# araffin/srl-zoo

Hardware: AMD Instinct MI355X
Metric: images/sec (224x224x3) AE+VAE train step (higher is better)
Workload: dtype f32; 1 GPU; synthetic 224x224x3 obs, --losses autoencoder, custom_cnn, state-dim 200, bs=256 per GPU (512 frames fwd+bwd per step per GPU), Adam lr 0.005, normalised fp32 observations resident in HBM; global_batch=256, parallelism=dp1, rccl_ranks=1, devices=1

## Files before the change

### include/srlz.h

```cpp
#ifndef SRLZ_H
#define SRLZ_H

#include <stddef.h>
#include <stdint.h>

#ifdef __cplusplus
extern "C" {
#endif

typedef void* srlz_stream_t;

enum srlz_status {
  SRLZ_OK = 0,
  SRLZ_ERR_BAD_DESC = -1,
  SRLZ_ERR_WORKSPACE = -2,
  SRLZ_ERR_HIP = -3,
  SRLZ_ERR_NULL = -4
};

#define SRLZ_ABI_VERSION 104
int srlz_version(void);
const char* srlz_last_error(void);
int srlz_device_cus(void);

typedef struct {
  int n;
  int hi, wi;
  int ho, wo;
  int ksize;
  int stride;
  int pad;
  int transposed;
  int groups;
} srlz_conv64_desc;

size_t srlz_conv64_packed_floats(void);
int srlz_conv64_pack_weights(const float* w_ref, float* wpack_fwd, float* wpack_bwd,
                             const srlz_conv64_desc* d, srlz_stream_t stream);
int srlz_conv64_fwd_tiles(const srlz_conv64_desc* d);
int srlz_conv64_fwd(const float* x, const float* wpack_fwd, const float* bias, float* y, float* stats_partial,
                    const float* x_bnp, const srlz_conv64_desc* d, srlz_stream_t stream);
typedef struct {
  const float* y;
  const float* bnp;
  const float* sums;
  long long count;
  int training;
  float* dy_out;
} srlz_bn_bwd_operand;
int srlz_conv64_bwd_data(const float* dy, const float* wpack_bwd, float* dx, const srlz_bn_bwd_operand* dy_bn,
                         const srlz_conv64_desc* d, srlz_stream_t stream);
struct srlz_pool_desc_s;
int srlz_conv64_bwd_data_tiles(const srlz_conv64_desc* d);
int srlz_conv64_bwd_data_pool_sums(const float* dy, const float* wpack_bwd, float* dx, const float* pooled, const float* pool_bnp,
                                   const float* pool_y, const uint8_t* pool_argmax, const struct srlz_pool_desc_s* pd,
                                   float* bn_bwd_partial, const srlz_conv64_desc* d, srlz_stream_t stream);
int srlz_conv64_bwd_fused_supported(const srlz_conv64_desc* d);
int srlz_conv64_gather_pipe_supported(const srlz_conv64_desc* d, int backward_data);
size_t srlz_conv64_bwd_fused_workspace(const srlz_conv64_desc* d);
int srlz_conv64_bwd_fused_bn_rows(const srlz_conv64_desc* d);
int srlz_conv64_bwd_fused(const float* x, const float* x_bnp, const float* dy, const srlz_bn_bwd_operand* dy_bn,
                          const float* wpack_bwd, float* dx, float* dw_ref, float* dbias ,
                          float* x_bn_bwd_partial , void* ws, size_t ws_bytes, const srlz_conv64_desc* d,
                          srlz_stream_t stream);
int srlz_conv64_wino_supported(const srlz_conv64_desc* d);
size_t srlz_conv64_wino_packed_floats(void);
int srlz_conv64_wino_pack_weights(const float* w_ref, float* upack_fwd, float* upack_bwd, srlz_stream_t stream);
int srlz_conv64_wino_tiles(const srlz_conv64_desc* d);
int srlz_conv64_wino_fwd(const float* x, const float* upack_fwd, const float* bias , float* y,
                         float* stats_partial , const float* x_bnp ,
                         const srlz_conv64_desc* d, srlz_stream_t stream);
int srlz_conv64_wino_bwd_data(const float* dy, const float* upack_bwd, float* dx, const srlz_conv64_desc* d, srlz_stream_t stream);
int srlz_conv64_wino_bwd_data_rows(const srlz_conv64_desc* d);
int srlz_conv64_wino_bwd_data_pool_sums(const float* dy, const float* upack_bwd, float* dx, const float* pooled, const float* pool_bnp,
                                        const float* pool_y, const uint8_t* pool_argmax, const struct srlz_pool_desc_s* pd,
                                        float* bn_bwd_partial, const srlz_conv64_desc* d, srlz_stream_t stream);
size_t srlz_conv64_wino_bwd_weight_workspace(const srlz_conv64_desc* d);
int srlz_conv64_wino_bwd_weight(const float* x, const float* dy, float* dw_ref, void* ws, size_t ws_bytes, const srlz_conv64_desc* d,
                                srlz_stream_t stream);
size_t srlz_conv64_bwd_weight_workspace(const srlz_conv64_desc* d);
int srlz_conv64_bwd_weight(const float* x, const float* dy, float* dw_ref, float* dbias, const float* x_bnp ,
                           const srlz_bn_bwd_operand* dy_bn ,
                           void* ws, size_t ws_bytes, const srlz_conv64_desc* d, srlz_stream_t stream);

typedef struct {
  int n, hi, wi, ho, wo;
  int cin, cout;
  int ksize, stride, pad;
  int groups;
} srlz_convn_desc;
size_t srlz_convn_packed_floats(const srlz_convn_desc* d);
int srlz_convn_pack_weights(const float* w_ref, float* wpack, const srlz_convn_desc* d, srlz_stream_t stream);
int srlz_convn_fwd_tiles(const srlz_convn_desc* d);
int srlz_convn_fwd(const float* x, const float* wpack, float* y, float* stats_partial, const float* x_bnp,
                   const srlz_convn_desc* d, srlz_stream_t stream);

typedef struct {
  int n;
  int c;
  int himg, wimg;
  int hf, wf;
  int kind;
  int groups;
} srlz_skinny_desc;

int srlz_skinny_tiles(const srlz_skinny_desc* d);
int srlz_conv1_fwd(const float* x_nchw, const float* w_ref, float* y_nhwc, float* stats_partial,
                   const srlz_skinny_desc* d, srlz_stream_t stream);
int srlz_conv1_fwd_u8(const uint8_t* x_u8, const float* norm_lut, const float* w_ref, float* y_nhwc, float* stats_partial,
                      const srlz_skinny_desc* d, srlz_stream_t stream);
size_t srlz_skinny_bwd_weight_workspace(const srlz_skinny_desc* d);
// ... 291 lines not shown
```

### srl-zoo_amd/csrc/conv64.hip

```cpp
#include "conv64_tile.h"
#include <stdlib.h>

static int floordiv(int a, int b) { return (a >= 0) ? a / b : -((-a + b - 1) / b); }

int conv64::build_program(Prog* P, int gather, int stride, int pad, int N, int Hs, int Ws, int Hd, int Wd, int G) {
  if (stride != 1 && stride != 2) return -1;
  if (G < 1 || N % G != 0) return -1;
  N /= G;
  P->N = N; P->Hs = Hs; P->Ws = Ws; P->Hd = Hd; P->Wd = Wd;
  P->G = G;
  P->src_gstride = (long long)N * Hs * Ws * 64;
  P->dst_gstride = (long long)N * Hd * Wd * 64;
  int kcls[3], kd[3];
  if (gather) {
    P->ss = stride; P->ds = 1;
    for (int k = 0; k < 3; ++k) {
      int t = k - pad;
      int c = ((t % stride) + stride) % stride;
      kcls[k] = c; kd[k] = (t - c) / stride;
    }
  } else {
    P->ss = 1; P->ds = stride;
    for (int k = 0; k < 3; ++k) {
      int py = (((k - pad) % stride) + stride) % stride;
// ... 355 lines not shown
                                                                    const float* __restrict__ wpack,
                                                                    const float* __restrict__ bias,
                                                                    float* __restrict__ dst,
                                                                    float* __restrict__ stats_partial,
                                                                    const ConvProg P, int ntiles, const OpFuse src_fuse_all) {
  conv64_fwd_body<NW, BWD, 0>(src, wpack, bias, dst, stats_partial, P, ntiles, src_fuse_all, SRLZ_NO_POOLSUM);
}

template <int PSUM>
__global__ __launch_bounds__(256, 2) void conv64_dgrad_poolsum_kernel(const float* __restrict__ src,
                                                                     const float* __restrict__ wpack,
                                                                     float* __restrict__ dst,
                                                                     float* __restrict__ bn_bwd_partial, const ConvProg P,
                                                                     int ntiles, const PoolSum ps) {
  conv64_fwd_body<4, false, PSUM>(src, wpack, nullptr, dst, bn_bwd_partial, P, ntiles, SRLZ_NO_FUSE, ps);
}

__global__ void conv64_pack_kernel(const float* __restrict__ w_ref, float* __restrict__ pf, float* __restrict__ pb,
                                   int transposed) {
  const int id = blockIdx.x * blockDim.x + threadIdx.x;
  if (id >= NTAPS * 4096) return;
  const int tap = id >> 12, n = (id >> 6) & 63, k = id & 63;
  const int o = (tap * 64 + n) * 64 + ((((k >> 2) ^ (n & 15)) << 2) | (k & 3));
  const int fwd_idx = transposed ? ((k * 64 + n) * 9 + tap) : ((n * 64 + k) * 9 + tap);
  const int bwd_idx = transposed ? ((n * 64 + k) * 9 + tap) : ((k * 64 + n) * 9 + tap);
  if (pf) pf[o] = w_ref[fwd_idx];
  if (pb) pb[o] = w_ref[bwd_idx];
}

static int check_desc(const srlz_conv64_desc* d) {
  SRLZ_REQUIRE(d != nullptr, SRLZ_ERR_NULL, "conv64: null descriptor");
  SRLZ_REQUIRE(d->ksize == 3 && (d->stride == 1 || d->stride == 2) && d->n > 0, SRLZ_ERR_BAD_DESC,
               "conv64: only 3x3 stride 1/2 supported (k=%d s=%d)", d->ksize, d->stride);
  SRLZ_REQUIRE(d->groups >= 0 && (d->groups <= 1 || d->n % d->groups == 0), SRLZ_ERR_BAD_DESC,
               "conv64: n = %d is not a multiple of groups = %d", d->n, d->groups);
  int eho, ewo;
  if (!d->transposed) {
    eho = (d->hi + 2 * d->pad - 3) / d->stride + 1;
    ewo = (d->wi + 2 * d->pad - 3) / d->stride + 1;
  } else {
    eho = (d->hi - 1) * d->stride - 2 * d->pad + 3;
    ewo = (d->wi - 1) * d->stride - 2 * d->pad + 3;
  }
  SRLZ_REQUIRE(eho == d->ho && ewo == d->wo, SRLZ_ERR_BAD_DESC, "conv64: output size %dx%d inconsistent (expected %dx%d)",
               d->ho, d->wo, eho, ewo);
  return 0;
}

static size_t fwd_lds_bytes(const ConvProg& P) {
  return (size_t)(TM + P.span) * 256 + 16384 + (size_t)64 * rowtab_passes(TM + P.span) + TM * 4 + 256 * 4;
}

static int launch_fwd(const float* src, const float* wpack, const float* bias, float* dst, float* stats,
                      const ConvProg& P, hipStream_t st, const OpFuse src_fuse = SRLZ_NO_FUSE, const PoolSum* psum = nullptr) {
  const int ntiles = P.G * P.tpg;
  const size_t lds = fwd_lds_bytes(P);
  SRLZ_REQUIRE(lds <= 160 * 1024, SRLZ_ERR_BAD_DESC, "conv64: tile needs %zu bytes of LDS", lds);
  SRLZ_REQUIRE(fits_32bit_src_floats(P) && fits_32bit_dst_rowinfo(P) && fits_31bit_grid(P, TM + P.span), SRLZ_ERR_BAD_DESC, "conv64: a group of %d images of %d x %d -> %d x %d is beyond the tile tables' 32-bit offsets", P.N, P.Hs,
               P.Ws, P.Hd, P.Wd);
  if (psum) {
    SRLZ_REQUIRE(!src_fuse.y && !src_fuse.bnp && stats && !bias, SRLZ_ERR_BAD_DESC, "conv64: the pooled-block epilogue takes a plain operand");
    bool one_class = true;
    for (int t = 1; t < NTAPS; ++t) one_class = one_class && P.tdst[t] == P.tdst[0];
    if (one_class) {
      SRLZ_MAX_LDS(conv64_dgrad_poolsum_kernel<1>, lds);
      SRLZ_LAUNCH(conv64_dgrad_poolsum_kernel<1>, dim3(ntiles), dim3(256), lds, st, src, wpack, dst, stats, P, ntiles, *psum);
    } else {
      SRLZ_MAX_LDS(conv64_dgrad_poolsum_kernel<2>, lds);
      SRLZ_LAUNCH(conv64_dgrad_poolsum_kernel<2>, dim3(ntiles), dim3(256), lds, st, src, wpack, dst, stats, P, ntiles, *psum);
    }
    return 0;
  }
#define SRLZ_FWD_LAUNCH(NWV, BWDV)                                                                                          \
  do {                                                                                                                     \
    SRLZ_MAX_LDS((conv64_fwd_kernel<NWV, BWDV>), lds);                                                                      \
    SRLZ_LAUNCH((conv64_fwd_kernel<NWV, BWDV>), dim3(ntiles), dim3(NWV * 64), lds, st, src, wpack, bias, dst, stats,        \
                P, ntiles, src_fuse);                                                                                      \
  } while (0)
  if (src_fuse.y) {
    SRLZ_REQUIRE(fits_32bit_src_floats(P), SRLZ_ERR_BAD_DESC,
                 "conv64: a group's operand has %lld floats (the fused staging keeps 32-bit row offsets)", (long long)P.N * P.Hs * P.Ws * 64);
    SRLZ_FWD_LAUNCH(4, true);
  } else {
    if (!src_fuse.bnp && !bias && conv64::gather_pipe_ok(P)) return conv64::launch_gather_pipe(src, wpack, dst, stats, P, st);
    SRLZ_FWD_LAUNCH(4, false);
  }
#undef SRLZ_FWD_LAUNCH
  return 0;
}

}

int conv64::with_program(const srlz_conv64_desc* d, int backward_data, Prog* P) {
  if (int rc = check_desc(d)) return rc;
  const int G = d->groups > 1 ? d->groups : 1;
  const int rc = backward_data ? build_program(P, d->transposed, d->stride, d->pad, d->n, d->ho, d->wo, d->hi, d->wi, G)
                               : build_program(P, !d->transposed, d->stride, d->pad, d->n, d->hi, d->wi, d->ho, d->wo, G);
  SRLZ_REQUIRE(rc == 0, SRLZ_ERR_BAD_DESC, "conv64: cannot build a grid program for this descriptor");
  return 0;
}

extern "C" size_t srlz_conv64_packed_floats(void) { return (size_t)NTAPS * 4096; }

extern "C" int srlz_conv64_pack_weights(const float* w_ref, float* wpack_fwd, float* wpack_bwd,
                                        const srlz_conv64_desc* d, srlz_stream_t stream) {
  if (int rc = check_desc(d)) return rc;
  SRLZ_REQUIRE(w_ref, SRLZ_ERR_NULL, "conv64_pack: null weights");
  SRLZ_LAUNCH(conv64_pack_kernel, dim3((NTAPS * 4096 + 255) / 256), dim3(256), 0, as_stream(stream), w_ref, wpack_fwd, wpack_bwd,
              d->transposed);
  return 0;
}

extern "C" int srlz_conv64_fwd_tiles(const srlz_conv64_desc* d) {
  ConvProg P;
  if (conv64::with_program(d, 0, &P)) return -1;
  return P.G * P.tpg;
}

extern "C" int srlz_conv64_fwd(const float* x, const float* wpack_fwd, const float* bias, float* y,
                               float* stats_partial, const float* x_bnp, const srlz_conv64_desc* d,
                               srlz_stream_t stream) {
  ConvProg P;
  if (int rc = conv64::with_program(d, 0, &P)) return rc;
  SRLZ_REQUIRE(x && wpack_fwd && y, SRLZ_ERR_NULL, "conv64_fwd: null pointer");
  return launch_fwd(x, wpack_fwd, bias, y, stats_partial, P, as_stream(stream), OpFuse{x_bnp, nullptr, nullptr, 0.f, 0, nullptr});
}

extern "C" int srlz_conv64_bwd_data(const float* dy, const float* wpack_bwd, float* dx, const srlz_bn_bwd_operand* dy_bn,
                                    const srlz_conv64_desc* d, srlz_stream_t stream) {
  ConvProg P;
  if (int rc = conv64::with_program(d, 1, &P)) return rc;
  SRLZ_REQUIRE(dy && wpack_bwd && dx, SRLZ_ERR_NULL, "conv64_bwd_data: null pointer");
  OpFuse gf;
  if (int rc = make_bwd_fuse(&gf, dy_bn, "conv64_bwd_data")) return rc;
  return launch_fwd(dy, wpack_bwd, nullptr, dx, nullptr, P, as_stream(stream), gf);
}

extern "C" int srlz_conv64_bwd_data_tiles(const srlz_conv64_desc* d) {
  ConvProg P;
  if (conv64::with_program(d, 1, &P)) return -1;
  return P.G * P.tpg;
}

extern "C" int srlz_conv64_bwd_data_pool_sums(const float* dy, const float* wpack_bwd, float* dx, const float* pooled,
                                              const float* pool_bnp, const float* pool_y, const uint8_t* pool_argmax,
                                              const srlz_pool_desc* pd, float* bn_bwd_partial, const srlz_conv64_desc* d,
                                              srlz_stream_t stream) {
  ConvProg P;
  if (int rc = conv64::with_program(d, 1, &P)) return rc;
  SRLZ_REQUIRE(dy && wpack_bwd && dx && pooled && pool_bnp && pool_y && pool_argmax && pd && bn_bwd_partial, SRLZ_ERR_NULL,
               "conv64_bwd_data_pool_sums: null pointer");
  SRLZ_REQUIRE(pd->n == d->n && pd->hp == d->hi && pd->wp == d->wi && !pd->out_nchw &&
               (pd->groups > 1 ? pd->groups : 1) == (d->groups > 1 ? d->groups : 1), SRLZ_ERR_BAD_DESC,
               "conv64_bwd_data_pool_sums: the pooled map [%d,%d,%d] is not this layer's input [%d,%d,%d]", pd->n, pd->hp, pd->wp, d->n,
               d->hi, d->wi);
  const int G = d->groups > 1 ? d->groups : 1;
  PoolSum ps = {pooled, pool_bnp, pool_y, pool_argmax, (long long)(pd->n / G) * pd->h * pd->w * 64, pd->h, pd->w, pd->pool_pad};
  return launch_fwd(dy, wpack_bwd, nullptr, dx, bn_bwd_partial, P, as_stream(stream), SRLZ_NO_FUSE, &ps);
}

extern "C" int srlz_conv64_debug_program(const srlz_conv64_desc* d, int backward_data, int* out, int cap) {
  ConvProg P;
  if (int rc = conv64::with_program(d, backward_data, &P)) return rc;
  if (cap < 12 + 4 * NTAPS) return SRLZ_ERR_WORKSPACE;
  int i = 0;
  out[i++] = P.N; out[i++] = P.PH; out[i++] = P.PW; out[i++] = P.ss; out[i++] = P.Hs; out[i++] = P.Ws;
  out[i++] = P.ds; out[i++] = P.Hd; out[i++] = P.Wd; out[i++] = P.min_off; out[i++] = P.span; out[i++] = P.s2;
  for (int t = 0; t < NTAPS; ++t) { out[i++] = P.tsrc[t]; out[i++] = P.tdst[t]; out[i++] = P.toff[t]; out[i++] = P.tw[t]; }
  return i;
}
```

### srl-zoo_amd/csrc/conv64_pipe.hip

```cpp
#include "conv64_tile.h"

namespace {

constexpr int GP_THREADS = 512;
constexpr int GP_RP = GP_THREADS / 16;
constexpr int GP_BATCH = 6;
constexpr int GP_CORE = TM / GP_RP;

struct GatherRows {
  f32x4 v[GP_BATCH], yv[GP_BATCH];
  unsigned offs[GP_CORE];
  unsigned ok;
};

constexpr int GT_P = 8;
constexpr int GT_WORDS = GP_RP * GT_P;
template <bool SHIFTED>
__device__ __forceinline__ void gtab_build(unsigned* __restrict__ tab, const ConvProg& P, int qstart, int nrows) {
  int R = threadIdx.x;
  asm volatile("" : "+v"(R));
  if (R < GT_WORDS) {
    unsigned e = 0;
    if (R < nrows) e = src_entry<SHIFTED>(P, qstart + R, 2);
    tab[(R & (GP_RP - 1)) * GT_P + (R >> 5)] = e;
// ... 612 lines not shown
    float* X = As0;
    if (wk == 1) {
#pragma unroll
      for (int r = 0; r < 16; ++r) X[((wave & 3) * 16 + r) * 64 + lane] = aw3[0][r];
    }
    __syncthreads();
    if (wk == 0) {
#pragma unroll
      for (int r = 0; r < 16; ++r) aw3[0][r] += X[((wave & 3) * 16 + r) * 64 + lane];
      put(aw3[0], 8, wmi, wnj);
    }
    __syncthreads();
    float* red = As0;
    *(f32x4*)(red + (tid >> 4) * 64 + (tid & 15) * 4) = bs4;
    __syncthreads();
    if (tid < 64) {
      float t = 0.f;
#pragma unroll
      for (int r = 0; r < GP_RP; ++r) t += red[r * 64 + tid];
      out[NTAPS * 4096 + tid] = t;
    }
  }
}

constexpr int BNZ_BLOCKS = 64;
__global__ __launch_bounds__(256) void conv64_bnpart_zero_scale_kernel(const float* __restrict__ x, const float* __restrict__ x_bnp,
                                                                      const float* __restrict__ da, float* __restrict__ bnpart,
                                                                      long long pixels, int bn_rows, int first_row) {
  const int g = blockIdx.y;
  x_bnp += g * 256;
  x += (size_t)g * pixels * 64;
  da += (size_t)g * pixels * 64;
  const int c4 = threadIdx.x & 15;
  const auto [mean, invstd, sc, sh] = load_bn_quads(x_bnp, c4);
  unsigned zmask = 0;
#pragma unroll
  for (int j = 0; j < 4; ++j) zmask |= (bnpart_zero_scale(sc[j], sh[j]) ? 1u : 0u) << j;
  double s1[4] = {0.0, 0.0, 0.0, 0.0}, s2[4] = {0.0, 0.0, 0.0, 0.0};
  if (__syncthreads_or(zmask != 0)) {
    for (long long pix = (long long)blockIdx.x * 16 + (threadIdx.x >> 4); pix < pixels; pix += (long long)gridDim.x * 16) {
      const f32x4 v = *(const f32x4*)(x + pix * 64 + c4 * 4);
      const f32x4 d = *(const f32x4*)(da + pix * 64 + c4 * 4);
#pragma unroll
      for (int j = 0; j < 4; ++j)
        if (((zmask >> j) & 1u) && v[j] * sc[j] + sh[j] > 0.f) {
          s1[j] += (double)d[j];
          s2[j] += (double)(d[j] * ((v[j] - mean[j]) * invstd[j]));
        }
    }
  }
  bn_bwd_combine_store(s1, s2, bnpart + ((size_t)g * bn_rows + first_row + blockIdx.x) * 128);
}

}

constexpr int GATHER_PIPE_MIN_TILES_PER_GROUP = 256;
bool conv64::gather_pipe_ok(const Prog& P) {
  if (P.tpg < GATHER_PIPE_MIN_TILES_PER_GROUP) return false;
  return taps_grouped_4221(P) && P.G <= 2 && fits_32bit_buffer_bytes(P) && TM + P.span <= GP_RP * GP_BATCH && GP_RP <= P.PHW &&
         -P.min_off <= P.PHW;
}

int conv64::launch_gather_pipe(const float* src, const float* wpack, float* dst, float* stats, const Prog& P, hipStream_t st) {
  const int ntiles = P.G * P.tpg;
  int pgrid = 2 * srlz_device_cus();
  if (pgrid > ntiles) pgrid = ntiles;
  pgrid &= ~7;
  if (pgrid < 8) pgrid = 8;
  const size_t plds = (size_t)(TM + P.span) * 256 + 16384 + 6 * TM * 4 + GT_WORDS * 4 + 8 * 64 * 4;
  SRLZ_MAX_LDS(conv64_gather_pipe_kernel, plds);
  SRLZ_LAUNCH(conv64_gather_pipe_kernel, dim3(pgrid), dim3(GP_THREADS), plds, st, src, wpack, dst, stats, ConvProg{P}, ntiles);
  return 0;
}

static bool fused_bwd_ok(const ConvProg& P) {
  const bool reach = P.toff[4] >= 0 && P.toff[5] >= 0 && P.toff[4] < FB_REACH1 && P.toff[5] < FB_REACH1 && P.toff[8] >= 0 &&
                     P.toff[8] <= FB_REACH3;
  return taps_grouped_4221(P) && P.G <= 2 && P.min_off == 0 && fits_32bit_buffer_bytes(P) && reach &&
         TM + P.span <= GP_RP * GP_BATCH && GP_RP <= P.PHW && P.G * P.tpg >= 8;
}

static int fused_bwd_grid(const ConvProg& P) {
  int g = srlz_device_cus() & ~7;
  const int ntiles = P.G * P.tpg;
  if (g > ntiles) g = (ntiles + 7) & ~7;
  return g;
}

extern "C" int srlz_conv64_gather_pipe_supported(const srlz_conv64_desc* d, int backward_data) {
  ConvProg P;
  if (conv64::with_program(d, backward_data, &P)) return 0;
  return conv64::gather_pipe_ok(P) ? 1 : 0;
}

extern "C" int srlz_conv64_bwd_fused_supported(const srlz_conv64_desc* d) {
  ConvProg P;
  if (conv64::with_program(d, 1, &P) || !d->transposed || d->stride != 2) return 0;
  return fused_bwd_ok(P) ? 1 : 0;
}

extern "C" int srlz_conv64_bwd_fused_bn_rows(const srlz_conv64_desc* d) {
  ConvProg P;
  if (conv64::with_program(d, 1, &P)) return -1;
  return P.G * (4 * P.tpg + BNZ_BLOCKS);
}

extern "C" size_t srlz_conv64_bwd_fused_workspace(const srlz_conv64_desc* d) {
  ConvProg P;
  if (conv64::with_program(d, 1, &P)) return 0;
  return (size_t)fused_bwd_grid(P) * WGRAD_PARTIAL_FLOATS * sizeof(float);
}

extern "C" int srlz_conv64_bwd_fused(const float* x, const float* x_bnp, const float* dy, const srlz_bn_bwd_operand* dy_bn,
                                     const float* wpack_bwd, float* dx, float* dw_ref, float* dbias, float* x_bn_bwd_partial,
                                     void* ws, size_t ws_bytes, const srlz_conv64_desc* d, srlz_stream_t stream) {
  ConvProg P;
  if (int rc = conv64::with_program(d, 1, &P)) return rc;
  SRLZ_REQUIRE(d->transposed && d->stride == 2, SRLZ_ERR_BAD_DESC, "conv64_bwd_fused: ConvTranspose2d(64, 64, 3, stride 2) only");
  SRLZ_REQUIRE(x && x_bnp && dy && dy_bn && wpack_bwd && dx && dw_ref && ws, SRLZ_ERR_NULL, "conv64_bwd_fused: null pointer");
  OpFuse gf;
  if (int rc = make_bwd_fuse(&gf, dy_bn, "conv64_bwd_fused")) return rc;
  SRLZ_REQUIRE(gf.dy_out == nullptr, SRLZ_ERR_BAD_DESC, "conv64_bwd_fused: d(loss)/dy is not materialised by this entry point");
  SRLZ_REQUIRE(fused_bwd_ok(P), SRLZ_ERR_BAD_DESC, "conv64_bwd_fused: shape not supported (ask srlz_conv64_bwd_fused_supported)");
  const int grid = fused_bwd_grid(P);
  SRLZ_REQUIRE(ws_bytes >= (size_t)grid * WGRAD_PARTIAL_FLOATS * sizeof(float), SRLZ_ERR_WORKSPACE,
// ... 18 lines not shown
```

### srl-zoo_amd/csrc/conv64_tile.h

```cpp
#pragma once
#include "common.h"

namespace {

#ifndef SRLZ_BATCH_FWD
#define SRLZ_BATCH_FWD 16
#endif
#ifndef SRLZ_BATCH_BWD
#define SRLZ_BATCH_BWD 12
#endif
constexpr int TM = 128;
constexpr int BATCH_FWD = SRLZ_BATCH_FWD;
constexpr int NTAPS = 9;
constexpr int WGRAD_PARTIAL_FLOATS = NTAPS * 4096 + 64;

}

namespace conv64 {

struct Prog {
  int N, PH, PW, PHW, total_q;
  int G, tpg;
  long long src_gstride, dst_gstride;
  int ss, Hs, Ws;
  int ds, Hd, Wd;
  int tsrc[NTAPS], tdst[NTAPS], toff[NTAPS], tw[NTAPS];
  int tp[NTAPS + 2];
  int min_off, span;
  int s2;
  int dbg;
  unsigned mPHW, mPW;
  int sPHW, sPW;
};

int build_program(Prog* P, int gather, int stride, int pad, int N, int Hs, int Ws, int Hd, int Wd, int G = 1);
int with_program(const srlz_conv64_desc* d, int backward_data, Prog* P);
bool gather_pipe_ok(const Prog& P);
int launch_gather_pipe(const float* src, const float* wpack, float* dst, float* stats, const Prog& P, hipStream_t st);
int launch_wgrad_reduce(const float* partial, int nwg, float* dw_ref, float* dbias, int transposed, int interleaved, hipStream_t st);

}

namespace {

struct ConvProg : conv64::Prog {};

struct OpFuse {
  const float* bnp;
  const float* y;
  const float* sums;
  float inv_count;
  int training;
  float* dy_out;
};
#define SRLZ_NO_FUSE OpFuse{nullptr, nullptr, nullptr, 0.f, 0, nullptr}

__device__ __forceinline__ OpFuse fuse_for_group(OpFuse f, int grp, long long goff) {
  if (f.bnp) f.bnp += grp * 256;
  if (f.sums) f.sums += grp * 128;
  if (f.y) f.y += goff;
  if (f.dy_out) f.dy_out += goff;
  return f;
}

struct GridPix { int n, y, x; };
template <bool SHIFTED>
__device__ __forceinline__ GridPix grid_pix(const ConvProg& P, int q, int stride) {
  const int qq = SHIFTED ? q + P.PHW : q;
  const int n1 = fastdiv(qq, P.mPHW, P.sPHW);
  const int rem = qq - n1 * P.PHW;
  const int a = fastdiv(rem, P.mPW, P.sPW);
  const int y = a * stride, x = (rem - a * P.PW) * stride;
  return GridPix{SHIFTED ? n1 - 1 : n1, y, x};
}

template <bool SHIFTED>
__device__ __forceinline__ unsigned src_entry(const ConvProg& P, int q, int ss) {
  const GridPix g = grid_pix<SHIFTED>(P, q, ss);
  if (SHIFTED ? (unsigned)g.n < (unsigned)P.N : g.n < P.N) {
    unsigned f = 0;
#pragma unroll
    for (int k = 0; k < 4; ++k) f |= (g.y + (k >> 1) < P.Hs && g.x + (k & 1) < P.Ws) ? 1u << k : 0u;
    return ((unsigned)((g.n * P.Hs + g.y) * P.Ws + g.x) << 4) | f;
  }
  return 0;
}

__device__ __forceinline__ unsigned pix_entry(int n, int y, int x, int H, int W) { return ((unsigned)((n * H + y) * W + x) << 1) | 1u; }

struct GridDiv { unsigned mPHW, mPW; int sPHW, sPW; };
__device__ __forceinline__ GridDiv grid_div(const ConvProg& P) { return GridDiv{P.mPHW, P.mPW, P.sPHW, P.sPW}; }
// ... 160 lines not shown
```

### srl-zoo_amd/srlz/_cabi.py

```python
import ctypes
import os
from ctypes import c_int, c_longlong, c_float, c_double, c_void_p, c_size_t, c_char_p, POINTER, Structure

_HERE = os.path.dirname(os.path.abspath(__file__))
LIB_PATH = os.path.join(_HERE, "libsrlz_hip.so")


ABI_VERSION = 104


class SrlzError(RuntimeError):
    pass


class Conv64Desc(Structure):
    _fields_ = [("n", c_int), ("hi", c_int), ("wi", c_int), ("ho", c_int), ("wo", c_int), ("ksize", c_int),
                ("stride", c_int), ("pad", c_int), ("transposed", c_int), ("groups", c_int)]


class SkinnyDesc(Structure):
    _fields_ = [("n", c_int), ("c", c_int), ("himg", c_int), ("wimg", c_int), ("hf", c_int), ("wf", c_int),
                ("kind", c_int), ("groups", c_int)]


class PoolDesc(Structure):
    _fields_ = [("n", c_int), ("h", c_int), ("w", c_int), ("hp", c_int), ("wp", c_int), ("pool_pad", c_int),
                ("out_nchw", c_int), ("groups", c_int)]


class ConvNDesc(Structure):
    _fields_ = [("n", c_int), ("hi", c_int), ("wi", c_int), ("ho", c_int), ("wo", c_int), ("cin", c_int), ("cout", c_int),
                ("ksize", c_int), ("stride", c_int), ("pad", c_int), ("groups", c_int)]

    def __init__(self, n, hi, wi, ho, wo, cin, cout, ksize, stride, pad, groups=1):
        super(ConvNDesc, self).__init__(n, hi, wi, ho, wo, cin, cout, ksize, stride, pad, groups)


class BnReplayItem(Structure):
    _fields_ = [("batch_stat", c_void_p), ("running_mean", c_void_p), ("running_var", c_void_p), ("num_batches_tracked", c_void_p)]


class BnBwdOperand(Structure):
    _fields_ = [("y", c_void_p), ("bnp", c_void_p), ("sums", c_void_p), ("count", c_longlong), ("training", c_int),
                ("dy_out", c_void_p)]


class InferBlockDesc(Structure):
    _fields_ = [("n", c_int), ("c_in", c_int), ("hi", c_int), ("wi", c_int), ("kind", c_int), ("pool_pad", c_int),
                ("out_nchw", c_int), ("stride_n", c_longlong), ("stride_c", c_longlong), ("stride_y", c_longlong),
                ("stride_x", c_longlong)]


INFER_IN, INFER_MID, INFER_LAST = 0, 1, 2

P = c_void_p
_BO = POINTER(BnBwdOperand)
_C64 = POINTER(Conv64Desc)
_SK = POINTER(SkinnyDesc)
_PD = POINTER(PoolDesc)
_CN = POINTER(ConvNDesc)
_IB = POINTER(InferBlockDesc)

_PROTOS = {
    "srlz_version": (c_int, []),
    "srlz_last_error": (c_char_p, []),
    "srlz_device_cus": (c_int, []),
    "srlz_conv64_packed_floats": (c_size_t, []),
    "srlz_conv64_pack_weights": (c_int, [P, P, P, _C64, P]),
    "srlz_conv64_fwd_tiles": (c_int, [_C64]),
    "srlz_conv64_fwd": (c_int, [P, P, P, P, P, P, _C64, P]),
    "srlz_conv64_bwd_data": (c_int, [P, P, P, _BO, _C64, P]),
    "srlz_conv64_bwd_weight_workspace": (c_size_t, [_C64]),
    "srlz_conv64_bwd_fused_supported": (c_int, [_C64]),
    "srlz_conv64_gather_pipe_supported": (c_int, [_C64, c_int]),
    "srlz_conv64_bwd_fused_workspace": (c_size_t, [_C64]),
    "srlz_conv64_bwd_fused": (c_int, [P, P, P, _BO, P, P, P, P, P, P, c_size_t, _C64, P]),
    "srlz_conv64_bwd_fused_bn_rows": (c_int, [_C64]),
    "srlz_conv64_wino_supported": (c_int, [_C64]),
    "srlz_conv64_wino_packed_floats": (c_size_t, []),
    "srlz_conv64_wino_pack_weights": (c_int, [P, P, P, P]),
    "srlz_conv64_wino_tiles": (c_int, [_C64]),
    "srlz_conv64_wino_fwd": (c_int, [P, P, P, P, P, P, _C64, P]),
    "srlz_conv64_wino_bwd_data": (c_int, [P, P, P, _C64, P]),
    "srlz_conv64_wino_bwd_weight_workspace": (c_size_t, [_C64]),
    "srlz_conv64_wino_bwd_weight": (c_int, [P, P, P, P, c_size_t, _C64, P]),
    "srlz_conv64_wino_bwd_data_rows": (c_int, [_C64]),
    "srlz_conv64_wino_bwd_data_pool_sums": (c_int, [P, P, P, P, P, P, P, _PD, P, _C64, P]),
    "srlz_conv64_bwd_weight": (c_int, [P, P, P, P, P, _BO, P, c_size_t, _C64, P]),
    "srlz_conv64_debug_program": (c_int, [_C64, c_int, POINTER(c_int), c_int]),
    "srlz_linear_debug_route": (c_int, [c_int, c_int, c_int, c_int, c_int, P, P, c_int, c_size_t, POINTER(c_int)]),
    "srlz_debug_placement": (c_int, [P, c_int, c_int, c_int, P]),
    "srlz_debug_mfma_peak": (c_int, [P, c_int, c_int, P]),
    "srlz_debug_mfma_valu": (c_int, [P, c_int, c_int, c_int, c_int, c_int, P]),
    "srlz_convn_packed_floats": (c_size_t, [_CN]),
    "srlz_convn_pack_weights": (c_int, [P, P, _CN, P]),
    "srlz_convn_fwd_tiles": (c_int, [_CN]),
    "srlz_convn_fwd": (c_int, [P, P, P, P, P, _CN, P]),
    "srlz_bn_finalize_chunks_workspace": (c_size_t, [c_int, c_int]),
    "srlz_bn_finalize_chunks": (c_int, [P, c_int, c_int, c_int, c_longlong, P, P, c_float, c_float, P, P, P, P, P, c_size_t, P]),
    "srlz_bn_eval_params_chunks": (c_int, [P, P, P, P, c_float, c_int, P, P]),
    "srlz_bn_add_relu": (c_int, [P, P, P, P, P, c_longlong, c_int, c_int, P]),
    "srlz_avgpool_nhwc": (c_int, [P, P, c_int, c_int, c_int, P]),
    "srlz_prelu_fwd": (c_int, [P, P, P, c_longlong, P]),
    "srlz_prelu_bwd": (c_int, [P, P, P, P, P, c_longlong, P]),
    "srlz_triplet_fwd": (c_int, [P, P, P, c_int, c_int, c_float, P, P, P]),
    "srlz_triplet_bwd": (c_int, [P, P, P, P, P, c_int, c_int, P, P, P, P]),
    "srlz_skinny_tiles": (c_int, [_SK]),
    "srlz_conv64_bwd_data_tiles": (c_int, [_C64]),
    "srlz_conv64_bwd_data_pool_sums": (c_int, [P, P, P, P, P, P, P, _PD, P, _C64, P]),
    "srlz_conv1_fwd": (c_int, [P, P, P, P, _SK, P]),
    "srlz_conv1_fwd_u8": (c_int, [P, P, P, P, P, _SK, P]),
    "srlz_conv1_bwd_weight_fused_u8": (c_int, [P, P, P, P, P, P, P, c_int, P, P, c_size_t, _SK, _PD, P]),
    "srlz_convT_out_fwd_loss_u8": (c_int, [P, P, P, P, P, P, P, P, P, _SK, P]),
    "srlz_normalize_lut": (c_int, [P, P]),
    "srlz_normalize_u8_planar": (c_int, [P, P, P, c_int, c_int, c_longlong, P]),
    "srlz_copy_frames_u8": (c_int, [P, P, c_longlong, P, P, c_longlong, c_int, c_longlong, P]),
    "srlz_copy_frames_u8_strided": (c_int, [P, P, c_longlong, c_longlong, c_longlong, P, P, c_longlong, c_longlong, c_longlong, c_int,
                                            c_longlong, P]),
    "srlz_occlude_frames_u8": (c_int, [P, P, c_longlong, P, P, P, c_int, c_int, c_int, c_int, P]),
    "srlz_skinny_bwd_weight_workspace": (c_size_t, [_SK]),
    "srlz_conv1_bwd_weight": (c_int, [P, P, P, P, c_size_t, _SK, P]),
    "srlz_conv1_bwd_data": (c_int, [P, P, P, _SK, P]),
    "srlz_conv1_bwd_weight_fused": (c_int, [P, P, P, P, P, P, c_int, P, P, c_size_t, _SK, _PD, P]),
    "srlz_bn_relu_pool_bwd_sums": (c_int, [P, P, P, P, P, P, P, P, P, c_size_t, _PD, P]),
    "srlz_convT_out_fwd": (c_int, [P, P, P, P, P, _SK, P]),
    "srlz_convT_out_bwd_data": (c_int, [P, P, P, P, P, P, _SK, P]),
    "srlz_bn_bwd_finalize_partials": (c_int, [P, c_int, c_int, P, P, P, P, c_size_t, P]),
# ... 57 lines not shown
    "srlz_reparam_fwd": (c_int, [P, P, P, P, c_longlong, P]),
    "srlz_reparam_bwd": (c_int, [P, P, P, P, P, c_longlong, P]),
    "srlz_cross_entropy": (c_int, [P, P, c_int, c_int, P, P, P]),
    "srlz_reward_prior_workspace": (c_size_t, [c_int]),
    "srlz_reward_prior_fwd": (c_int, [P, P, c_int, c_int, P, P, c_size_t, P]),
    "srlz_reward_prior_bwd": (c_int, [P, P, P, c_size_t, P, c_int, c_int, P, P]),
    "srlz_episode_prior_workspace": (c_size_t, [c_int, c_int]),
    "srlz_episode_prior_fwd": (c_int, [P, P, P, c_int, c_int, P, P, P, P, P, P, P, P, c_size_t, P, P]),
    "srlz_episode_prior_bwd": (c_int, [P, P, P, P, c_int, c_int, P, P, P, P, c_size_t, P, P, P, P, P, P, P, P]),
    "srlz_knn_workspace": (c_size_t, [c_int, c_int, c_int, c_int]),
    "srlz_knn_f64": (c_int, [P, c_int, P, c_int, c_int, c_int, P, P, P, c_size_t, P]),
    "srlz_gtc_workspace": (c_size_t, [c_int, c_int, c_int]),
    "srlz_gtc_rows_f64": (c_int, [P, P, c_int, c_int, c_int, P, P, P, c_size_t, P]),
    "srlz_reward_probe_chunk_rows": (c_int, [c_int]),
    "srlz_reward_probe_fit": (c_int, [P, P, c_int, c_int, P, P, c_int, c_int, P, P, P, c_int, c_double, c_double, c_double, c_double, P,
                                      P, P, P]),
    "srlz_reward_probe_eval_workspace": (c_size_t, [c_int, c_int]),
    "srlz_reward_probe_eval": (c_int, [P, P, c_int, c_int, P, P, c_int, c_int, P, P, P, P, c_size_t, P, P]),
    "srlz_decoded_to_bgr": (c_int, [P, c_int, c_int, c_int, P, P]),
    "srlz_decoded_to_sheet_u8": (c_int, [P, c_int, c_int, c_int, c_int, c_int, c_int, c_int, P, c_int, c_int, P]),
    "srlz_pca_workspace": (c_size_t, [c_int, c_int]),
    "srlz_pca_transform_workspace": (c_size_t, [c_int, c_int, c_int]),
    "srlz_pca_stats": (c_int, [P, P, P, c_int, c_int, c_int, c_longlong, P, P, P, P, P]),
    "srlz_pca_gram": (c_int, [P, c_int, c_int, P, P, P, c_int, c_int, P, P, c_int, P, P, c_size_t, P]),
    "srlz_pca_project": (c_int, [P, P, c_int, c_int, P, P, P, c_int, c_int, P, P, c_int, P, P]),
    "srlz_pca_transform": (c_int, [P, P, P, c_int, c_int, P, P, P, c_int, c_int, P, P, c_size_t, P]),
    "srlz_mse_target_fwd": (c_int, [P, P, c_int, c_int, P, P, P]),
    "srlz_dropout_fwd": (c_int, [P, P, c_float, P, c_int, c_int, P]),
    "srlz_dropout_bwd": (c_int, [P, P, c_float, P, c_int, c_int, P]),
    "srlz_concat_onehot": (c_int, [P, P, P, c_int, c_int, c_int, P]),
    "srlz_normalize_u8": (c_int, [P, P, c_int, c_int, c_int, c_int, P]),
    "srlz_mask_columns": (c_int, [P, P, c_int, c_int, c_int, c_int, P]),
    "srlz_param_norms": (c_int, [P, P, c_int, c_int, c_float, P, P, P]),
    "srlz_param_norms_grad": (c_int, [P, P, P, c_int, c_int, P, P, c_float, P]),
    "srlz_fold_grads": (c_int, [P, P, c_longlong, c_int, P]),
    "srlz_comm_unique_id_bytes": (c_size_t, []),
    "srlz_comm_unique_id": (c_int, [P]),
    "srlz_comm_init": (c_int, [P, c_int, c_int]),
    "srlz_comm_world": (c_int, []),
    "srlz_comm_allreduce_f32": (c_int, [P, c_longlong, P]),
    "srlz_comm_destroy": (c_int, []),
    "srlz_adam_step": (c_int, [P, P, P, P, c_longlong, c_double, c_double, c_double, c_double, c_int, c_float, P]),
    "srlz_adam_step_dev": (c_int, [P, P, P, P, c_longlong, c_double, c_double, c_double, c_double, P, P, c_float, P]),
    "srlz_infer_block_supported": (c_int, [_IB]),
    "srlz_infer_block_out_dims": (c_int, [_IB, POINTER(c_int), POINTER(c_int), POINTER(c_int), POINTER(c_int)]),
    "srlz_infer_tile": (c_int, []),
    "srlz_infer_packed_floats": (c_longlong, [c_int, c_int]),
    "srlz_infer_pack_weights": (c_int, [P, P, c_int, c_int, P]),
    "srlz_infer_block": (c_int, [P, P, P, P, P, _IB, P]),
}

_NOT_STATUS = {"srlz_version", "srlz_device_cus", "srlz_conv64_fwd_tiles", "srlz_skinny_tiles", "srlz_convn_fwd_tiles",
               "srlz_convT_out_bwd_fused_tiles", "srlz_convT_out_fwd_loss_workgroups", "srlz_conv64_bwd_fused_supported", "srlz_conv64_gather_pipe_supported",
               "srlz_convT_out_bwd_fused_supported",
               "srlz_conv64_bwd_data_tiles", "srlz_conv64_bwd_fused_bn_rows", "srlz_conv64_wino_supported", "srlz_conv64_wino_packed_floats",
               "srlz_conv64_wino_tiles", "srlz_conv64_wino_bwd_data_rows",
               "srlz_conv64_debug_program", "srlz_comm_world", "srlz_dense_supported",
               "srlz_dense_out_fwd_loss_workgroups", "srlz_reward_probe_chunk_rows", "srlz_infer_block_supported",
               "srlz_infer_tile"}

EXPORTED = sorted(_PROTOS.keys())


def _load():
    if not os.path.exists(LIB_PATH):
        raise SrlzError(
            "libsrlz_hip.so not found at %s — build it with `python -c 'import __graft_entry__ as g; g.build()'` "
            "(or `make -C srl-zoo_amd/csrc`). There is no CPU fallback for the srl-zoo_amd hot path." % LIB_PATH)
    lib = ctypes.CDLL(LIB_PATH)
    for name, (res, args) in _PROTOS.items():
        fn = getattr(lib, name)
        fn.restype = res
        fn.argtypes = args
    got = lib.srlz_version()
    if got != ABI_VERSION:
        raise SrlzError("libsrlz_hip.so at %s reports ABI version %d, these bindings are written for %d (include/srlz.h "
                        "SRLZ_ABI_VERSION): rebuild with `make -C srl-zoo_amd/csrc`" % (LIB_PATH, got, ABI_VERSION))
    return lib


_lib = _load()


def error_text():
    return _lib.srlz_last_error().decode("utf-8", "replace")


_DEBUG_SYNC = bool(os.environ.get("SRLZ_SYNC"))


def _wrap(name):
    fn = getattr(_lib, name)
    if _PROTOS[name][0] is c_int and name not in _NOT_STATUS:
        def call(*a):
            rc = fn(*a)
            if rc != 0:
                raise SrlzError("%s failed (%d): %s" % (name, rc, error_text()))
            if _DEBUG_SYNC:
                import torch
                torch.cuda.synchronize()
            return rc
        call.__name__ = name
        return call
    return fn


# ... 14 lines not shown
```

Baseline: 44550 images/s.

## Add persistent scatter-pipe kernel for stride-2 transposed conv64 forward

Adds a persistent, XCD-aware scatter-pipeline kernel for the forward pass of stride-2 scatter-style (transposed) 64-channel convolutions. It prefetches the next tile's source rows into registers during the current tile's MFMA loop and double-buffers the row tables. It also fuses the BN+ReLU prologue, bias and stats epilogue, and flushes each output parity class as its taps complete. The aim is to hide global-load latency and launch/tile overhead that the generic forward kernel exposes. In exchange it adds a large new code path with tight eligibility conditions and higher register pressure.

```diff
diff --git a/include/srlz.h b/include/srlz.h
--- a/include/srlz.h
+++ b/include/srlz.h
@@ -57,6 +57,7 @@
                                    float* bn_bwd_partial, const srlz_conv64_desc* d, srlz_stream_t stream);
 int srlz_conv64_bwd_fused_supported(const srlz_conv64_desc* d);
 int srlz_conv64_gather_pipe_supported(const srlz_conv64_desc* d, int backward_data);
+int srlz_conv64_scatter_pipe_supported(const srlz_conv64_desc* d, int backward_data);
 size_t srlz_conv64_bwd_fused_workspace(const srlz_conv64_desc* d);
 int srlz_conv64_bwd_fused_bn_rows(const srlz_conv64_desc* d);
 int srlz_conv64_bwd_fused(const float* x, const float* x_bnp, const float* dy, const srlz_bn_bwd_operand* dy_bn,
diff --git a/srl-zoo_amd/csrc/conv64.hip b/srl-zoo_amd/csrc/conv64.hip
--- a/srl-zoo_amd/csrc/conv64.hip
+++ b/srl-zoo_amd/csrc/conv64.hip
@@ -431,7 +431,8 @@
 }
 
 static int launch_fwd(const float* src, const float* wpack, const float* bias, float* dst, float* stats,
-                      const ConvProg& P, hipStream_t st, const OpFuse src_fuse = SRLZ_NO_FUSE, const PoolSum* psum = nullptr) {
+                      const ConvProg& P, hipStream_t st, const OpFuse src_fuse = SRLZ_NO_FUSE, const PoolSum* psum = nullptr,
+                      bool forward = false) {
   const int ntiles = P.G * P.tpg;
   const size_t lds = fwd_lds_bytes(P);
   SRLZ_REQUIRE(lds <= 160 * 1024, SRLZ_ERR_BAD_DESC, "conv64: tile needs %zu bytes of LDS", lds);
@@ -462,6 +463,7 @@
     SRLZ_FWD_LAUNCH(4, true);
   } else {
     if (!src_fuse.bnp && !bias && conv64::gather_pipe_ok(P)) return conv64::launch_gather_pipe(src, wpack, dst, stats, P, st);
+    if (forward && conv64::scatter_pipe_ok(P)) return conv64::launch_scatter_pipe(src, wpack, bias, dst, stats, src_fuse.bnp, P, st);
     SRLZ_FWD_LAUNCH(4, false);
   }
 #undef SRLZ_FWD_LAUNCH
@@ -502,7 +504,8 @@
   ConvProg P;
   if (int rc = conv64::with_program(d, 0, &P)) return rc;
   SRLZ_REQUIRE(x && wpack_fwd && y, SRLZ_ERR_NULL, "conv64_fwd: null pointer");
-  return launch_fwd(x, wpack_fwd, bias, y, stats_partial, P, as_stream(stream), OpFuse{x_bnp, nullptr, nullptr, 0.f, 0, nullptr});
+  return launch_fwd(x, wpack_fwd, bias, y, stats_partial, P, as_stream(stream), OpFuse{x_bnp, nullptr, nullptr, 0.f, 0, nullptr}, nullptr,
+                    true);
 }
 
 extern "C" int srlz_conv64_bwd_data(const float* dy, const float* wpack_bwd, float* dx, const srlz_bn_bwd_operand* dy_bn,
diff --git a/srl-zoo_amd/csrc/conv64_pipe.hip b/srl-zoo_amd/csrc/conv64_pipe.hip
--- a/srl-zoo_amd/csrc/conv64_pipe.hip
+++ b/srl-zoo_amd/csrc/conv64_pipe.hip
@@ -688,6 +688,261 @@
   bn_bwd_combine_store(s1, s2, bnpart + ((size_t)g * bn_rows + first_row + blockIdx.x) * 128);
 }
 
+constexpr int SP_THREADS = 256;
+constexpr int SP_RP = SP_THREADS / 16;
+constexpr int SP_BATCH = 12;
+constexpr int ST_WORDS = SP_RP * SP_BATCH;
+
+struct ScatterRows {
+  f32x4 v[SP_BATCH];
+  unsigned ok;
+};
+
+__device__ __forceinline__ void stab_build(unsigned* __restrict__ tab, const ConvProg& P, int qstart, int nrows) {
+  int R = threadIdx.x;
+  asm volatile("" : "+v"(R));
+  if (R < ST_WORDS) {
+    unsigned e = 0;
+    if (R < nrows) e = src_entry<true>(P, qstart + R, P.ss);
+    tab[(R & (SP_RP - 1)) * SP_BATCH + (R >> 4)] = e;
+  }
+}
+
+__device__ __forceinline__ void scatter_request(ScatterRows& r, const float* __restrict__ src, const unsigned* __restrict__ tab) {
+  int t = threadIdx.x;
+  asm volatile("" : "+v"(t));
+  const int slot = t & 15;
+  const unsigned* __restrict__ tp = tab + (t >> 4) * SP_BATCH;
+  const uint4 e0 = *(const uint4*)tp, e1 = *(const uint4*)(tp + 4), e2 = *(const uint4*)(tp + 8);
+  const unsigned e[SP_BATCH] = {e0.x, e0.y, e0.z, e0.w, e1.x, e1.y, e1.z, e1.w, e2.x, e2.y, e2.z, e2.w};
+  static_assert(SP_BATCH == 12, "the table read above takes twelve rows");
+  unsigned okmask = 0;
+#pragma unroll
+  for (int j = 0; j < SP_BATCH; ++j) {
+    const unsigned m = (unsigned)__builtin_amdgcn_sbfe((int)e[j], 0u, 1u);
+    const unsigned off = (((e[j] >> 4) << 6) & m) + slot * 4;
+    r.v[j] = *(const f32x4*)(src + off);
+    okmask |= m & (1u << j);
+  }
+  r.ok = okmask;
+}
+
+template <bool FUSE>
+__device__ __forceinline__ void scatter_land(float* __restrict__ lds, ScatterRows& r, int nrows, const float* __restrict__ lrec) {
+  int t = threadIdx.x;
+  asm volatile("" : "+v"(t));
+  const int slot = t & 15;
+  f32x4 sc4 = {1.f, 1.f, 1.f, 1.f}, sh4 = {0.f, 0.f, 0.f, 0.f};
+  if constexpr (FUSE) { sc4 = *(const f32x4*)(lrec + slot * 4); sh4 = *(const f32x4*)(lrec + 64 + slot * 4); }
+#pragma unroll
+  for (int j = 0; j < SP_BATCH; ++j) {
+    const int R = (t >> 4) + SP_RP * j;
+    const bool ok = (r.ok >> j) & 1u;
+    f32x4 v = r.v[j];
+    if constexpr (FUSE) {
+#pragma unroll
+      for (int e = 0; e < 4; ++e) { const float z = __builtin_fmaf(v[e], sc4[e], sh4[e]); v[e] = z > 0.f ? z : 0.f; }
+    }
+    if (!ok) v = f32x4{0.f, 0.f, 0.f, 0.f};
+    if (j < TM / SP_RP || R < nrows) *(f32x4*)(lds + R * 64 + ((slot ^ (R & 15)) << 2)) = v;
+  }
+}
+
+__device__ __forceinline__ void scatter_flush(const f32x16 (&acc)[2], const float (&bcol)[2], float* __restrict__ S,
+                                              const float* __restrict__ zero4, const int* __restrict__ ri,
+                                              const __amdgpu_buffer_rsrc_t dst, int d, int Wd, f32x4& s4, f32x4& q4) {
+  int tid_f = threadIdx.x;
+  asm volatile("" : "+v"(tid_f));
+  const int lane = tid_f & 63, wrow = tid_f >> 6;
+  const int h = lane >> 5, l31 = lane & 31;
+  const int need = d >> 1 | (d & 1) << 1;
+  const unsigned ddelta = (unsigned)((d >> 1) * Wd + (d & 1));
+  const int eg = lane >> 4, eslot = lane & 15;
+#pragma unroll
+  for (int half = 0; half < 2; ++half) {
+#pragma unroll
+    for (int rr = 0; rr < 8; ++rr) {
+      const int rowl = (rr & 3) + 8 * (rr >> 2) + 4 * h;
+      const int swz = (rowl & 4) << 3;
+#pragma unroll
+      for (int j = 0; j < 2; ++j) S[rowl * 64 + ((32 * j + l31) ^ swz)] = acc[j][8 * half + rr] + bcol[j];
+    }
+#pragma unroll
+    for (int k = 0; k < 4; ++k) {
+      const int rowl = eg + 4 * k;
+      const int row = wrow * 32 + 16 * half + rowl;
+      const int w = ri[row];
+      const bool inside = w >= 0 && (w & need) == need;
+      const f32x4 v = *(const f32x4*)(inside ? S + rowl * 64 + ((eslot ^ ((rowl & 4) << 1)) << 2) : zero4);
+      __builtin_amdgcn_raw_buffer_store_b128(v, dst, inside ? ((unsigned)(w >> 2) + ddelta) * 256u + eslot * 16 : GP_DROP, 0, 0);
+#pragma unroll
+      for (int e = 0; e < 4; ++e) { s4[e] += v[e]; q4[e] = __builtin_fmaf(v[e], v[e], q4[e]); }
+    }
+  }
+}
+
+template <bool FUSE>
+__global__ __launch_bounds__(SP_THREADS, 2) void conv64_scatter_pipe_kernel(const float* __restrict__ src_all,
+                                                                           const float* __restrict__ wpack,
+                                                                           const float* __restrict__ bias,
+                                                                           float* __restrict__ dst_all,
+                                                                           float* __restrict__ stats_partial, const ConvProg P,
+                                                                           int ntiles, const float* __restrict__ bnp_all) {
+  extern __shared__ __attribute__((aligned(16))) unsigned char smem[];
+  float* As = (float*)smem;
+  float* Bs = As + (TM + P.span) * 64;
+  int* rowinfo = (int*)(Bs + 4096);
+  unsigned* stab = (unsigned*)(rowinfo + 2 * TM);
+  float* frec = (float*)(stab + ST_WORDS);
+  float* red = frec + 256;
+  float* zero4 = red + 512;
+
+  const int tid = threadIdx.x;
+  const int lane = tid & 63, wave = tid >> 6;
+  const int nrows = TM + P.span;
+  const int d0 = P.tdst[0], d1 = P.tdst[4], d2 = P.tdst[6], d3 = P.tdst[8];
+
+  const int xcd = blockIdx.x & 7, wi = blockIdx.x >> 3, wpx = gridDim.x >> 3;
+  const int tq = ntiles >> 3, tr = ntiles & 7;
+  const int tbase = (xcd < tr) ? xcd * (tq + 1) : tr * (tq + 1) + (xcd - tr) * tq;
+  const int tcnt = tq + (xcd < tr ? 1 : 0);
+
+  if (tid < 4) zero4[tid] = 0.f;
+  if constexpr (FUSE) {
+    if (tid < 64 * P.G) {
+      const int g = tid >> 6, c = tid & 63;
+      frec[g * 128 + c] = bnp_all[g * 256 + 128 + c];
+      frec[g * 128 + 64 + c] = bnp_all[g * 256 + 192 + c];
+    }
+  }
+  float bcol[2];
+#pragma unroll
+  for (int j = 0; j < 2; ++j) bcol[j] = bias ? bias[j * 32 + (lane & 31)] : 0.f;
+
+  constexpr int BV = 1024 / SP_THREADS;
+  f32x4 breg[BV];
+  {
+    const f32x4* wsrc = (const f32x4*)(wpack + (size_t)P.tw[0] * 4096);
+#pragma unroll
+    for (int i = 0; i < BV; ++i) breg[i] = wsrc[wave * (BV * 64) + lane + i * 64];
+  }
+  const unsigned dst_bytes = (unsigned)P.dst_gstride * 4u;
+
+  ScatterRows rr;
+  int k = wi;
+  int parity = 0;
+  if (k < tcnt) {
+    const int tile = tbase + k;
+    const int grp = (P.G > 1 && tile >= P.tpg) ? 1 : 0;
+    const int q0 = (tile - grp * P.tpg) * TM;
+    stab_build(stab, P, q0 + P.min_off, nrows);
+    __syncthreads();
+    scatter_request(rr, src_all + grp * P.src_gstride, stab);
+    scatter_land<FUSE>(As, rr, nrows, frec + grp * 128);
+  }
+  for (; k < tcnt; k += wpx, parity ^= 1) {
+    const int tile = tbase + k;
+    const int grp = (P.G > 1 && tile >= P.tpg) ? 1 : 0;
+    const int q0 = (tile - grp * P.tpg) * TM;
+    const __amdgpu_buffer_rsrc_t dst = raw_buffer(dst_all + grp * P.dst_gstride, dst_bytes);
+    const int k2 = k + wpx;
+    const int tile2 = tbase + (k2 < tcnt ? k2 : k);
+    const int grp2 = (P.G > 1 && tile2 >= P.tpg) ? 1 : 0;
+    const int q02 = (tile2 - grp2 * P.tpg) * TM;
+    int* ri = rowinfo + parity * TM;
+    if (tid < TM) {
+      const int q = q0 + tid;
+      int w = -1;
+      if (q < P.total_q) {
+        const GridPix g = grid_pix<false>(P, q, P.ds);
+        if (g.y < P.Hd && g.x < P.Wd) w = (((g.n * P.Hd + g.y) * P.Wd + g.x) << 2) | (g.y + 1 < P.Hd ? 1 : 0) | (g.x + 1 < P.Wd ? 2 : 0);
+      }
+      ri[tid] = w;
+    }
+    f32x16 acc[2];
+    f32x4 s4 = {0.f, 0.f, 0.f, 0.f}, q4 = {0.f, 0.f, 0.f, 0.f};
+    int tid_t = tid;
+    asm volatile("" : "+v"(tid_t));
+    const int lane_t = tid_t & 63, wave_t = tid_t >> 6;
+    const int h_t = lane_t >> 5, l31_t = lane_t & 31;
+    const int arow0 = wave_t * 32 + l31_t - P.min_off;
+    const float* brow = Bs + l31_t * 64;
+    const int bkey = lane_t & 15;
+    const int bslot_t = wave_t * (BV * 64) + lane_t;
+    float* S = Bs + wave_t * 1024;
+
+#pragma unroll
+    for (int ti = 0; ti < NTAPS; ++ti) {
+      constexpr f32x16 zero16 = {0.f, 0.f, 0.f, 0.f, 0.f, 0.f, 0.f, 0.f, 0.f, 0.f, 0.f, 0.f, 0.f, 0.f, 0.f, 0.f};
+      const bool first = ti == 0 || ti == 4 || ti == 6 || ti == 8;
+      __syncthreads();
+      if (ti == 4) scatter_flush(acc, bcol, S, zero4, ri, dst, d0, P.Wd, s4, q4);
+      if (ti == 6) scatter_flush(acc, bcol, S, zero4, ri, dst, d1, P.Wd, s4, q4);
+      if (ti == 8) scatter_flush(acc, bcol, S, zero4, ri, dst, d2, P.Wd, s4, q4);
+      {
+        f32x4* wdst = (f32x4*)Bs;
+#pragma unroll
+        for (int i = 0; i < BV; ++i) wdst[bslot_t + i * 64] = breg[i];
+      }
+      {
+        const f32x4* wsrc = (const f32x4*)(wpack + (size_t)P.tw[(ti + 1) % NTAPS] * 4096);
+#pragma unroll
+        for (int i = 0; i < BV; ++i) breg[i] = wsrc[bslot_t + i * 64];
+      }
+      if (ti == 6) stab_build(stab, P, q02 + P.min_off, k2 < tcnt ? nrows : 0);
+      __syncthreads();
+      if (ti == 7) scatter_request(rr, src_all + grp2 * P.src_gstride, stab);
+      __builtin_amdgcn_sched_barrier(0);
+      const int R = arow0 + P.toff[ti];
+      int abase = (R * 64 + ((h_t ^ (R & 15)) << 2)) * 4;
+      asm volatile("" : "+v"(abase));
+      f32x4 a = *(const f32x4*)((const char*)As + abase);
+      f32x4 b[2];
+#pragma unroll
+      for (int j = 0; j < 2; ++j) b[j] = *(const f32x4*)(brow + j * 2048 + ((h_t ^ bkey) << 2));
+#pragma unroll
+      for (int kc = 0; kc < 8; ++kc) {
+        f32x4 an = a, bn[2] = {b[0], b[1]};
+        if (kc < 7) {
+          an = *(const f32x4*)((const char*)As + (abase ^ ((kc + 1) << 5)));
+#pragma unroll
+          for (int j = 0; j < 2; ++j) bn[j] = *(const f32x4*)(brow + j * 2048 + ((((kc + 1) * 2 + h_t) ^ bkey) << 2));
+        }
+        __builtin_amdgcn_sched_barrier(0);
+#pragma unroll
+        for (int r = 0; r < 4; ++r)
+#pragma unroll
+          for (int j = 0; j < 2; ++j)
+            acc[j] = __builtin_amdgcn_mfma_f32_32x32x2f32(a[r], b[j][r], (first && kc == 0 && r == 0) ? zero16 : acc[j], 0, 0, 0);
+        a = an;
+        b[0] = bn[0]; b[1] = bn[1];
+      }
+    }
+    __syncthreads();
+    scatter_land<FUSE>(As, rr, nrows, frec + grp2 * 128);
+    scatter_flush(acc, bcol, S, zero4, ri, dst, d3, P.Wd, s4, q4);
+    if (stats_partial) {
+      int tid_s = tid;
+      asm volatile("" : "+v"(tid_s));
+      const int lane_s = tid_s & 63, wrow_s = tid_s >> 6;
+#pragma unroll
+      for (int e = 0; e < 4; ++e) {
+        s4[e] += __shfl_xor(s4[e], 16, 64); s4[e] += __shfl_xor(s4[e], 32, 64);
+        q4[e] += __shfl_xor(q4[e], 16, 64); q4[e] += __shfl_xor(q4[e], 32, 64);
+      }
+      if (lane_s < 16) {
+        *(f32x4*)(red + wrow_s * 128 + lane_s * 4) = s4;
+        *(f32x4*)(red + wrow_s * 128 + 64 + lane_s * 4) = q4;
+      }
+      __syncthreads();
+      if (tid_s < 128) {
+        const float v = red[tid_s] + red[128 + tid_s] + red[256 + tid_s] + red[384 + tid_s];
+        stats_partial[(size_t)tile * 128 + tid_s] = v;
+      }
+    }
+  }
+}
+
 }
 
 constexpr int GATHER_PIPE_MIN_TILES_PER_GROUP = 256;
@@ -707,6 +962,41 @@
   SRLZ_MAX_LDS(conv64_gather_pipe_kernel, plds);
   SRLZ_LAUNCH(conv64_gather_pipe_kernel, dim3(pgrid), dim3(GP_THREADS), plds, st, src, wpack, dst, stats, ConvProg{P}, ntiles);
   return 0;
+}
+
+constexpr int SCATTER_PIPE_MIN_TILES_PER_GROUP = 256;
+bool conv64::scatter_pipe_ok(const Prog& P) {
+  if (P.tpg < SCATTER_PIPE_MIN_TILES_PER_GROUP) return false;
+  bool grouped = P.s2 && P.ss == 1 && P.ds == 2 && !P.dbg;
+  for (int t = 0; t < NTAPS; ++t) grouped = grouped && P.tsrc[t] == 0 && P.tdst[t] == P.tdst[t < 4 ? 0 : t < 6 ? 4 : t < 8 ? 6 : 8];
+  return grouped && P.G <= 2 && fits_32bit_buffer_bytes(P) && fits_32bit_src_floats(P) && fits_32bit_dst_rowinfo(P) &&
+         fits_31bit_grid(P, TM + P.span) && TM + P.span <= SP_RP * SP_BATCH && -P.min_off <= P.PHW;
+}
+
+int conv64::launch_scatter_pipe(const float* src, const float* wpack, const float* bias, float* dst, float* stats, const float* bnp,
+                                const Prog& P, hipStream_t st) {
+  const int ntiles = P.G * P.tpg;
+  int pgrid = 2 * srlz_device_cus();
+  if (pgrid > ntiles) pgrid = ntiles;
+  pgrid &= ~7;
+  if (pgrid < 8) pgrid = 8;
+  const size_t plds = (size_t)(TM + P.span) * 256 + 16384 + 2 * TM * 4 + ST_WORDS * 4 + 256 * 4 + 512 * 4 + 16;
+  if (bnp) {
+    SRLZ_MAX_LDS(conv64_scatter_pipe_kernel<true>, plds);
+    SRLZ_LAUNCH(conv64_scatter_pipe_kernel<true>, dim3(pgrid), dim3(SP_THREADS), plds, st, src, wpack, bias, dst, stats, ConvProg{P},
+                ntiles, bnp);
+  } else {
+    SRLZ_MAX_LDS(conv64_scatter_pipe_kernel<false>, plds);
+    SRLZ_LAUNCH(conv64_scatter_pipe_kernel<false>, dim3(pgrid), dim3(SP_THREADS), plds, st, src, wpack, bias, dst, stats, ConvProg{P},
+                ntiles, bnp);
+  }
+  return 0;
+}
+
+extern "C" int srlz_conv64_scatter_pipe_supported(const srlz_conv64_desc* d, int backward_data) {
+  ConvProg P;
+  if (backward_data || conv64::with_program(d, 0, &P)) return 0;
+  return conv64::scatter_pipe_ok(P) ? 1 : 0;
 }
 
 static bool fused_bwd_ok(const ConvProg& P) {
diff --git a/srl-zoo_amd/csrc/conv64_tile.h b/srl-zoo_amd/csrc/conv64_tile.h
--- a/srl-zoo_amd/csrc/conv64_tile.h
+++ b/srl-zoo_amd/csrc/conv64_tile.h
@@ -37,6 +37,9 @@
 int with_program(const srlz_conv64_desc* d, int backward_data, Prog* P);
 bool gather_pipe_ok(const Prog& P);
 int launch_gather_pipe(const float* src, const float* wpack, float* dst, float* stats, const Prog& P, hipStream_t st);
+bool scatter_pipe_ok(const Prog& P);
+int launch_scatter_pipe(const float* src, const float* wpack, const float* bias, float* dst, float* stats, const float* bnp,
+                        const Prog& P, hipStream_t st);
 int launch_wgrad_reduce(const float* partial, int nwg, float* dw_ref, float* dbias, int transposed, int interleaved, hipStream_t st);
 
 }
diff --git a/srl-zoo_amd/srlz/_cabi.py b/srl-zoo_amd/srlz/_cabi.py
--- a/srl-zoo_amd/srlz/_cabi.py
+++ b/srl-zoo_amd/srlz/_cabi.py
@@ -73,6 +73,7 @@
     "srlz_conv64_bwd_weight_workspace": (c_size_t, [_C64]),
     "srlz_conv64_bwd_fused_supported": (c_int, [_C64]),
     "srlz_conv64_gather_pipe_supported": (c_int, [_C64, c_int]),
+    "srlz_conv64_scatter_pipe_supported": (c_int, [_C64, c_int]),
     "srlz_conv64_bwd_fused_workspace": (c_size_t, [_C64]),
     "srlz_conv64_bwd_fused": (c_int, [P, P, P, _BO, P, P, P, P, P, P, c_size_t, _C64, P]),
     "srlz_conv64_bwd_fused_bn_rows": (c_int, [_C64]),
@@ -236,6 +237,7 @@
 
 _NOT_STATUS = {"srlz_version", "srlz_device_cus", "srlz_conv64_fwd_tiles", "srlz_skinny_tiles", "srlz_convn_fwd_tiles",
                "srlz_convT_out_bwd_fused_tiles", "srlz_convT_out_fwd_loss_workgroups", "srlz_conv64_bwd_fused_supported", "srlz_conv64_gather_pipe_supported",
+               "srlz_conv64_scatter_pipe_supported",
                "srlz_convT_out_bwd_fused_supported",
                "srlz_conv64_bwd_data_tiles", "srlz_conv64_bwd_fused_bn_rows", "srlz_conv64_wino_supported", "srlz_conv64_wino_packed_floats",
                "srlz_conv64_wino_tiles", "srlz_conv64_wino_bwd_data_rows",
```

Result: faster. 45060 images/s, median of 6 (+1.2%).
